# hongfz16/Garment4D

Hardware: AMD Instinct MI355X
Metric: point-cloud frames/s (FPS+ball_query+SA-MLP+LBS), B=8 N=8192 (higher is better)
Workload: dtype f32

## Files before the change

### garment4d_amd/_lib.py

```python
import ctypes
import os

_HERE = os.path.dirname(os.path.abspath(__file__))
LIB_PATH = os.environ.get("G4D_LIB_PATH") or os.path.join(_HERE, "lib", "libg4d_hip.so")

_vp = ctypes.c_void_p
_I = ctypes.c_int
_F = ctypes.c_float
_LL = ctypes.c_longlong

SIGNATURES = {
    "g4d_fps_f32": [_I, _I, _I, _vp, _vp, _vp, _vp],
    "g4d_fps_gather_f32": [_I, _I, _I, _vp, _vp, _vp, _vp, _vp],
    "g4d_gather_f32": [_I, _I, _I, _I, _vp, _vp, _vp, _vp],
    "g4d_gather_grad_f32": [_I, _I, _I, _I, _vp, _vp, _vp, _vp],
    "g4d_ball_query_f32": [_I, _I, _I, _F, _I, _vp, _vp, _vp, _vp],
    "g4d_ball_query_msg_f32": [_I, _I, _I, _I, _vp, _vp, _vp, _vp, _vp, _vp],
    "g4d_ball_query_boxes_f32": [_I, _I, _I, _I, _vp, _vp, _vp, _vp, _vp, _vp, _vp],
    "g4d_ball_query_lanes_f32": [_I, _I, _I, _I, _vp, _vp, _vp, _vp, _vp, _vp, _vp, _vp],
    "g4d_ball_query_lanes_qsort_bytes": [_I, _I],
    "g4d_ball_grid_bytes": [_I, _I],
    "g4d_ball_grid_build_f32": [_I, _I, _F, _vp, _vp, _vp],
    "g4d_ball_grid_query_f32": [_I, _I, _I, _I, _vp, _vp, _vp, _vp, _vp, _vp, _F, _vp],
    "g4d_ball_query_grid_f32": [_I, _I, _I, _I, _vp, _vp, _vp, _vp, _vp, _vp, _vp],
# ... 48 lines not shown
    "g4d_mlp_chain_table_f32": [ctypes.c_longlong, _I, _I, _I, _vp, _vp, _vp, _vp, _vp, _vp, _I, _I, _vp, _vp, _vp, _vp, _vp, _vp, _vp, _I, _I, _I, _vp, _I, _vp],
    "g4d_mlp_chain_group_table_f32": [ctypes.c_longlong, _I, _I, _I, _vp, _vp, _vp, _vp, _I, _I, _vp, _vp, _vp, _I, _vp, _vp, _vp, _vp, _vp, _vp, _I, _vp, _I, _I, _vp],
    "g4d_mlp_args_size": [],
    "g4d_mlp_run": [_I, _vp, _vp],
    "g4d_sa_table_supported": [ctypes.c_longlong, _I, _I, _I],
    "g4d_sa_table_ws_bytes": [ctypes.c_longlong, _I, _I, _I],
    "g4d_mlp_chain_group_table_ws_f32": [ctypes.c_longlong, _I, _I, _I, _vp, _vp, _vp, _vp, _I, _I, _vp, _vp, _vp, _I, _vp, _vp, _vp, _vp, _vp, _vp, _I, _vp, _I, _I, _vp,
                                         ctypes.c_longlong, _vp],
    "g4d_three_nn_cells_f32": [_I, _I, _I, _vp, _vp, _vp, _vp, _vp, _vp],
    "g4d_mlp_chain_interp_init_f32": [ctypes.c_longlong, _I, _I, _I, _vp, _vp, _I, _vp, _vp, _I, _vp, _vp, _vp, _vp, _vp, _vp, _vp, _I, _I, _I, _vp, _I, _vp],
    "g4d_three_nn_multi_f32": [_I, _I, _vp, _vp, _vp, _vp, _vp, _vp, _vp],
    "g4d_ball_query_msg2_f32": [_I, _I, _I, _I, _vp, _vp, _vp, _vp, _vp, _I, _I, _vp, _vp, _vp, _vp, _vp, _vp],
    "g4d_fps_gather_pair_supported": [_I, _I, _I],
    "g4d_fps_gather_pair_f32": [_I, _I, _I, _I, _vp, _vp, _vp, _vp, _vp, _vp],
    "g4d_sa_xyz_mlp3_pair_f32": [_I, _I, _I, _vp, _vp, _I, _vp, _I, _I, _vp, _vp, _I, _vp, _vp, _vp, _I, _vp, _vp, _vp, _I, _vp, _vp, _I, _I, _vp, _vp, _I, _vp, _vp, _vp, _I, _vp, _vp, _vp, _I, _vp, _vp, _I, _vp],
    "g4d_fps_gather_grid_f32": [_I, _I, _I, _vp, _vp, _vp, ctypes.c_float, _vp, _vp],
    "g4d_three_nn_cells_sorted_f32": [_I, _I, _I, _vp, _vp, _vp, _vp, _vp],
    "g4d_three_nn_pruned_supported": [_I, _I],
    "g4d_three_nn_pruned_ws_bytes": [_I],
    "g4d_three_nn_pruned_f32": [_I, _I, _I, _vp, _vp, _vp, _vp, _vp, _I, _vp, ctypes.c_longlong, _vp],
    "g4d_mlp_chain_table_cells_f32": [ctypes.c_longlong, _I, _I, _I, _vp, _vp, _vp, _vp, _vp, _vp, _vp, _I, _I, _vp, _vp, _vp, _vp, _vp, _vp, _vp, _I, _I, _I, _vp, _I, _vp],
    "g4d_search_multi_f32": [_I, _I, _I, _I, _vp, _vp, _vp, _vp, _vp, _I, _I, _vp, _vp, _vp, _vp, _vp, _I, _vp, _vp, _vp, _vp, _vp, _vp, _vp],
    "g4d_launch_group_begin": [],
    "g4d_launch_group_end": [_vp, _vp],
    "g4d_launch_group_abort": [],
    "g4d_lbs_one_supported": [_I, _I],
    "g4d_lbs_one_f32": [_I, _I, _I, _I, _I, _vp, _I, _vp, _vp, _vp, _vp, _vp, _vp, _vp, _vp, _vp, _vp, _vp],
    "g4d_lbs_mfma_supported": [_I, _I],
    "g4d_lbs_mfma_ws_bytes": [_I, _I],
    "g4d_lbs_mfma_f32": [_I, _I, _I, _I, _I, _vp, _I, _vp, _vp, _vp, _vp, _vp, _vp, _vp, _vp, _vp, _vp, _vp, ctypes.c_longlong, _vp],
# ... 2 lines not shown
    "g4d_segment_take_f32": [_I, _I, _I, _I, _vp, _vp, _vp, _vp],
    "g4d_vertex_normals_f32": [_I, _I, _vp, _vp, _vp, _vp, _vp, _vp],
    "g4d_spmm_axpy_rows_f32": [_I, _I, _I, _vp, _vp, _vp, _vp, _F, _vp, _vp],
    "g4d_jacobi_smooth_f32": [_I, _I, _I, _I, _F, _I, _vp, _vp, _vp, _vp, _vp, _vp],
    "g4d_gather_rows_f32": [_I, _I, _I, _I, _vp, _vp, _vp, _vp],
    "g4d_lbs_shape_f32": [_I, _I, _I, _vp, _I, _vp, _vp, _vp, _vp],
    "g4d_joint_regress_f32": [_I, _I, _I, _vp, _I, _vp, _vp, _vp],
    "g4d_rodrigues_f32": [_I, _vp, _vp, _vp],
    "g4d_rigid_transform_f32": [_I, _I, _I, _vp, _vp, _vp, _vp, _vp, _vp, _vp, _vp],
    "g4d_lbs_pose_skin_f32": [_I, _I, _I, _I, _vp, _vp, _vp, _vp, _I, _vp, _vp, _vp, _vp],
}

_lib = None


RESTYPES = {"g4d_mlp_args_size": ctypes.c_uint, "g4d_sa_table_ws_bytes": ctypes.c_longlong, "g4d_gcn_tile_meta_bytes": ctypes.c_longlong, "g4d_frag_bf16_elems": ctypes.c_longlong, "g4d_lbs_mfma_ws_bytes": ctypes.c_longlong, "g4d_three_nn_pruned_ws_bytes": ctypes.c_longlong, "g4d_temporal_attention_scratch_floats": ctypes.c_size_t, "g4d_ball_grid_bytes": ctypes.c_size_t, "g4d_ball_query_lanes_qsort_bytes": ctypes.c_size_t}


class G4DError(RuntimeError):
    pass


MLP_ARGS_VERSION = 1
MLP_STACK_F32, MLP_STACK_BF16, MLP_WAVE_F32, MLP_CHAIN_F32, MLP_CHAIN_BF16, MLP_CHAIN_BF16X3 = range(6)


class MlpArgs(ctypes.Structure):
    _fields_ = [("size", ctypes.c_uint), ("version", ctypes.c_uint), ("mode", _I), ("K0", _I), ("rows", ctypes.c_longlong),
                ("X", _vp), ("ldx", _I),
                ("N", _I), ("P", _I), ("S", _I), ("C", _I), ("use_xyz", _I), ("xyz", _vp), ("new_xyz", _vp), ("feats", _vp), ("idx", _vp),
                ("n", _I), ("m", _I), ("C2", _I), ("C1", _I), ("known_feats", _vp), ("skip", _vp), ("dist2", _vp), ("nn_idx", _vp),
# ... 105 lines not shown
```

### garment4d_amd/csrc/api.hip

```cpp
#include <stdarg.h>
#include <stddef.h>
#include <stdlib.h>
#include <string.h>

#include "g4d_common.h"

namespace g4d {
static thread_local char g_err[512] = "";

void set_error(const char *fmt, ...) {
    va_list ap;
    va_start(ap, fmt);
    vsnprintf(g_err, sizeof(g_err), fmt, ap);
    va_end(ap);
}

static int g_contract = -1;

static int parse_contract(const char *e) {
    if (!e || !*e) return G4D_CONTRACT_NVCC;
    if (!strcmp(e, "0") || !strcmp(e, "off") || !strcmp(e, "none")) return G4D_CONTRACT_OFF;
    if (!strcmp(e, "2") || !strcmp(e, "chain") || !strcmp(e, "inner")) return G4D_CONTRACT_CHAIN;
    return G4D_CONTRACT_NVCC;
}
// ... 4 lines not shown
    if (t_contract >= 0) return t_contract;
    int m = __atomic_load_n(&g_contract, __ATOMIC_RELAXED);
    if (m < 0) {
        m = parse_contract(getenv("G4D_DIST_CONTRACT"));
        __atomic_store_n(&g_contract, m, __ATOMIC_RELAXED);
    }
    return m;
}
}

namespace g4d {
namespace {
struct Tune { const char *key; long long value; int state; };
Tune g_tune[] = {{"sa_table_persistent", 0, 0}, {"sa_table_min_rows", 0, 0}, {"sa_table_128", 0, 0}, {"sa_table_oversub", 0, 0}, {"sa_table_dedup", 0, 0}, {"fp_table_persistent", 0, 0},
                 {"fp_table_min_rows", 0, 0}, {"gemm_tile", 0, 0}, {"gemm_tile_min_rows", 0, 0}, {"gemm_tile_min_cout", 0, 0}, {"gemm_tile_min_kpad", 0, 0}, {"fp_init_persistent", 0, 0}, {"fp_init_min_rows", 0, 0},
                 {"fp_head_bf16_persistent", 0, 0}, {"fp_head_bf16_min_rows", 0, 0}, {"sa_group_bf16_persistent", 0, 0}, {"sa_group_bf16_min_rows", 0, 0}};
}
struct ThreadTune { long long value; bool set; };
thread_local ThreadTune t_tune[sizeof(g_tune) / sizeof(g_tune[0])] = {};

long long tuning(const char *key, long long dflt) {
    int i = 0;
    for (Tune &t : g_tune) {
        const int slot = i++;
        if (strcmp(t.key, key)) continue;
        if (t_tune[slot].set) return t_tune[slot].value;
        int st = __atomic_load_n(&t.state, __ATOMIC_ACQUIRE);
        if (st == 0) {
            char env[64] = "G4D_";
            size_t n = 4;
            for (const char *c = key; *c && n + 1 < sizeof(env); ++c) env[n++] = (char)((*c >= 'a' && *c <= 'z') ? *c - 32 : *c);
// ... 32 lines not shown
    if (key) {
        int i = 0;
        for (g4d::Tune &t : g4d::g_tune) {
            const int slot = i++;
            if (!strcmp(t.key, key)) {
                g4d::t_tune[slot].value = value;
                g4d::t_tune[slot].set = set != 0;
                return G4D_OK;
            }
        }
    }
    g4d::set_error("g4d_tuning_set_thread: unknown key '%s'", key ? key : "(null)");
    return G4D_EINVAL;
}

extern "C" int g4d_version(void) { return 260;  }
extern "C" const char *g4d_last_error(void) { return g4d::g_err; }

extern "C" int g4d_get_distance_contraction(void) { return g4d::distance_contraction(); }
extern "C" int g4d_set_distance_contraction_thread(int mode) {
    const int prev = g4d::t_contract;
    if (mode < -1 || mode > G4D_CONTRACT_CHAIN) {
        g4d::set_error("g4d_set_distance_contraction_thread: mode %d is not -1 (no override) or one of G4D_CONTRACT_OFF/NVCC/CHAIN", mode);
        return -2;
    }
    g4d::t_contract = mode;
    return prev;
}

extern "C" int g4d_set_distance_contraction(int mode) {
    const int saved = g4d::t_contract;
// ... 97 lines not shown
```

### garment4d_amd/csrc/sa_xyz.hip

```cpp
#include <cstdlib>

#include "g4d_common.h"

namespace g4d {

typedef float f32x4 __attribute__((ext_vector_type(4)));

struct SaXyzArgs {
    int n, p, S, logS, pool;
    long long rows;
    const float *xyz, *new_xyz;
    const int *idx;
    const float *W1, *sc1, *sh1;
    int ldw1;
    const float *W2f, *sc2, *sh2;
    const float *W3f, *sc3, *sh3;
    int kst2, kst3;
    float *out;
    int ldo, col0;
};

struct __attribute__((packed, aligned(4))) F3s { float x, y, z; };
__device__ __forceinline__ F3s ld3(const float *base, unsigned elem) {
    return *reinterpret_cast<const F3s *>(reinterpret_cast<const char *>(base) + (elem << 2));
}

__device__ __forceinline__ float pool4_rows_max(float v0, float v1, float v2, float v3) {
    const auto a = __builtin_amdgcn_permlane16_swap(__float_as_uint(v0), __float_as_uint(v1), false, false);
    const auto b = __builtin_amdgcn_permlane16_swap(__float_as_uint(v2), __float_as_uint(v3), false, false);
    const float m01 = fmaxf(__uint_as_float(a[0]), __uint_as_float(a[1]));
    const float m23 = fmaxf(__uint_as_float(b[0]), __uint_as_float(b[1]));
    const auto c = __builtin_amdgcn_permlane32_swap(__float_as_uint(m01), __float_as_uint(m23), false, false);
    return fmaxf(__uint_as_float(c[0]), __uint_as_float(c[1]));
}

template <int C1, int C2, int C3, int LOGS, bool MAXP>
__device__ __forceinline__ void sa_xyz_body(const SaXyzArgs &a, int first, int stride) {
    constexpr int T1 = C1 / 16, T2 = C2 / 16, T3 = C3 / 16;
    constexpr int S = 1 << LOGS;
    static_assert(S == 16 || S == 32, "16 or 32 samples");
    static_assert(T3 == 2 || T3 == 4, "32 or 64 output channels");
    const int lane = threadIdx.x & 63;
    const int fi = lane & 15, fq = lane >> 4;
    float w1f[T1], s1[T1][4], h1s[T1][4];
#pragma unroll
    for (int ks = 0; ks < T1; ++ks) {
        const float w = a.W1[(ks * 16 + fi) * a.ldw1 + min(fq, 2)];
        w1f[ks] = fq < 3 ? w : 0.f;
#pragma unroll
        for (int e = 0; e < 4; ++e) {
            const int c = ks * 16 + fq * 4 + e;
// ... 9 lines not shown
#pragma unroll
    for (int ct = 0; ct < T3; ++ct)
#pragma unroll
        for (int ks = 0; ks < T2; ++ks) w3[ct][ks] = *reinterpret_cast<const f32x4 *>(a.W3f + ((size_t)(ct * a.kst3 + ks) * 64 + lane) * 4);
    f32x4 s2[T2], h2s[T2];
#pragma unroll
    for (int ct = 0; ct < T2; ++ct) {
        s2[ct] = *reinterpret_cast<const f32x4 *>(a.sc2 + ct * 16 + fq * 4);
        h2s[ct] = *reinterpret_cast<const f32x4 *>(a.sh2 + ct * 16 + fq * 4);
    }
    float s3[T3], h3s[T3];
#pragma unroll
    for (int ct = 0; ct < T3; ++ct) { s3[ct] = a.sc3[ct * 16 + fi]; h3s[ct] = a.sh3[ct * 16 + fi]; }

    const int rows = (int)a.rows;
    const int npass = (rows + 31) >> 5;
    struct Rows { float px[2], pq[2]; };
    int ivn[2];
    auto load_idx = [&](int pass, int (&v)[2]) {
#pragma unroll
        for (int mt = 0; mt < 2; ++mt) v[mt] = a.idx[min(min(pass, npass - 1) * 32 + mt * 16 + fi, rows - 1)];
    };
    const int nq = (int)(a.rows >> LOGS);
    auto load_rows = [&](int pass, const int (&v)[2], Rows &rw) {
        pass = min(pass, npass - 1);
#pragma unroll
        for (int mt = 0; mt < 2; ++mt) {
            const int qi = __builtin_amdgcn_readfirstlane(min((pass * 32 + mt * 16) >> LOGS, nq - 1));
            const int f = qi / a.p;
            rw.px[mt] = a.xyz[(unsigned)(f * a.n + v[mt]) * 3u + cfq];
            rw.pq[mt] = a.new_xyz[(unsigned)qi * 3u + cfq];
        }
    };
    auto do_pass = [&](int pass, const Rows &cur, Rows &fill, bool alive) {
        load_rows(pass + stride, ivn, fill);
        load_idx(pass + 2 * stride, ivn);
        __builtin_amdgcn_sched_barrier(0);
        const int row0 = pass * 32;
        f32x4 h1[2][T1];
#pragma unroll
        for (int mt = 0; mt < 2; ++mt) {
            const float d = cur.px[mt] - cur.pq[mt];
            const float comp = fq < 3 ? d : 0.f;
#pragma unroll
            for (int ks = 0; ks < T1; ++ks) {
                const f32x4 acc = __builtin_amdgcn_mfma_f32_16x16x4f32(w1f[ks], comp, (f32x4){0.f, 0.f, 0.f, 0.f}, 0, 0, 0);
#pragma unroll
                for (int e = 0; e < 4; ++e) h1[mt][ks][e] = fmaxf(__builtin_fmaf(acc[e], s1[ks][e], h1s[ks][e]), 0.f);
            }
// ... 20 lines not shown
                for (int r = 0; r < 4; ++r) h2[mt][ct][r] = fmaxf(__builtin_fmaf(h2[mt][ct][r], s2[ct][r], h2s[ct][r]), 0.f);
        f32x4 acc[2][T3];
#pragma unroll
        for (int mt = 0; mt < 2; ++mt)
#pragma unroll
            for (int ct = 0; ct < T3; ++ct) acc[mt][ct] = (f32x4){0.f, 0.f, 0.f, 0.f};
#pragma unroll
        for (int ks = 0; ks < T2; ++ks)
#pragma unroll
            for (int e = 0; e < 4; ++e)
#pragma unroll
                for (int mt = 0; mt < 2; ++mt)
#pragma unroll
                    for (int ct = 0; ct < T3; ++ct)
                        acc[mt][ct] = __builtin_amdgcn_mfma_f32_16x16x4f32(h2[mt][ks][e], w3[ct][ks][e], acc[mt][ct], 0, 0, 0);
        if constexpr (MAXP) {
            float v[2][T3];
#pragma unroll
            for (int mt = 0; mt < 2; ++mt)
#pragma unroll
                for (int ct = 0; ct < T3; ++ct) {
                    const float y0 = __builtin_fmaf(acc[mt][ct][0], s3[ct], h3s[ct]), y1 = __builtin_fmaf(acc[mt][ct][1], s3[ct], h3s[ct]),
                                y2 = __builtin_fmaf(acc[mt][ct][2], s3[ct], h3s[ct]), y3 = __builtin_fmaf(acc[mt][ct][3], s3[ct], h3s[ct]);
                    v[mt][ct] = fmaxf(fmaxf(y0, y1), fmaxf(y2, y3));
                }
            if constexpr (S == 32) {
                float x[T3];
#pragma unroll
                for (int ct = 0; ct < T3; ++ct) x[ct] = fmaxf(v[0][ct], v[1][ct]);
                float *o = a.out + (size_t)pass * a.ldo + a.col0;
                if constexpr (T3 == 4) {
// ... 66 lines not shown
        if (a.S == 16) sa_xyz_body<C1, C2, C3, 4, false>(a, first, stride);
        else sa_xyz_body<C1, C2, C3, 5, false>(a, first, stride);
    }
}

template <int C1, int C2, int C3>
__global__ void __launch_bounds__(256, 2) sa_xyz_kernel(const SaXyzArgs a) {
    sa_xyz_dispatch<C1, C2, C3>(a, blockIdx.x * 4 + __builtin_amdgcn_readfirstlane(threadIdx.x >> 6), gridDim.x * 4);
}

template <bool MAXP>
__global__ void __launch_bounds__(256, 2) sa_xyz_pair_kernel(const SaXyzArgs a0, const SaXyzArgs a1) {
    const int first = blockIdx.x * 4 + __builtin_amdgcn_readfirstlane(threadIdx.x >> 6), stride = gridDim.x * 4;
    sa_xyz_body<32, 32, 64, 5, MAXP>(a1, first, stride);
    sa_xyz_body<16, 16, 32, 4, MAXP>(a0, first, stride);
}

}

using namespace g4d;

extern "C" int g4d_sa_xyz_mlp3_supported(int c1, int c2, int c3, int nsample) {
    return ((c1 == 16 && c2 == 16 && c3 == 32) || (c1 == 32 && c2 == 32 && c3 == 64)) && (nsample == 16 || nsample == 32);
}

static int sa_xyz_fill(SaXyzArgs &a, int b, int n, int p, int nsample, const float *xyz, const float *new_xyz, const int *idx, int c1, int c2, int c3,
                       const float *W1, int ldw1, const float *scale1, const float *shift1, const float *W2_frag, int kpad2, const float *scale2,
                       const float *shift2, const float *W3_frag, int kpad3, const float *scale3, const float *shift3, int pool, float *out, int ldo,
                       int col0) {
    G4D_REQUIRE(b >= 0 && n > 0 && p >= 0, "g4d_sa_xyz_mlp3_f32: bad sizes");
    G4D_REQUIRE(g4d_sa_xyz_mlp3_supported(c1, c2, c3, nsample), "g4d_sa_xyz_mlp3_f32: widths %d-%d-%d over %d samples are not instantiated", c1, c2,
                c3, nsample);
    G4D_REQUIRE(pool == 1 || pool == 2, "g4d_sa_xyz_mlp3_f32: pool must be 1 (max) or 2 (avg)");
    const long long rows = (long long)b * p * nsample;
    G4D_REQUIRE(xyz && new_xyz && idx && W1 && scale1 && shift1 && W2_frag && scale2 && shift2 && W3_frag && scale3 && shift3 && out && ldw1 >= 3,
                "g4d_sa_xyz_mlp3_f32: null pointer");
    G4D_REQUIRE(ldo >= col0 + c3 && col0 >= 0, "g4d_sa_xyz_mlp3_f32: output window out of range");
    G4D_REQUIRE(rows < (1ll << 31) - 64 && (long long)b * n * 12 < (1ll << 32), "g4d_sa_xyz_mlp3_f32: needs rows < 2^31 and b*n*12 B < 4 GB");
    a.n = n; a.p = p; a.S = nsample; a.logS = nsample == 16 ? 4 : 5; a.pool = pool; a.rows = rows;
    a.xyz = xyz; a.new_xyz = new_xyz; a.idx = idx; a.W1 = W1; a.sc1 = scale1; a.sh1 = shift1; a.ldw1 = ldw1;
    G4D_REQUIRE(kpad2 % 16 == 0 && kpad2 >= c1 && kpad3 % 16 == 0 && kpad3 >= c2, "g4d_sa_xyz_mlp3_f32: Kpad of layers 2 / 3 must be multiples of 16 covering c1 / c2");
    a.W2f = W2_frag; a.sc2 = scale2; a.sh2 = shift2; a.W3f = W3_frag; a.sc3 = scale3; a.sh3 = shift3; a.kst2 = kpad2 / 16; a.kst3 = kpad3 / 16;
    a.out = out; a.ldo = ldo; a.col0 = col0;
    return G4D_OK;
}

extern "C" int g4d_sa_xyz_mlp3_pair_f32(int b, int n, int p, const float *xyz, const float *new_xyz, int pool, float *out, int ldo,
                                        int nsample0, const int *idx0, const float *W1_0, int ldw1_0, const float *scale1_0, const float *shift1_0,
                                        const float *W2_frag0, int kpad2_0, const float *scale2_0, const float *shift2_0, const float *W3_frag0,
                                        int kpad3_0, const float *scale3_0, const float *shift3_0, int col0_0,
                                        int nsample1, const int *idx1, const float *W1_1, int ldw1_1, const float *scale1_1, const float *shift1_1,
                                        const float *W2_frag1, int kpad2_1, const float *scale2_1, const float *shift2_1, const float *W3_frag1,
                                        int kpad3_1, const float *scale3_1, const float *shift3_1, int col0_1, g4d_stream_t stream) {
    SaXyzArgs a0, a1;
    if (int rc = sa_xyz_fill(a0, b, n, p, nsample0, xyz, new_xyz, idx0, 16, 16, 32, W1_0, ldw1_0, scale1_0, shift1_0, W2_frag0, kpad2_0, scale2_0, shift2_0,
                             W3_frag0, kpad3_0, scale3_0, shift3_0, pool, out, ldo, col0_0)) return rc;
    if (int rc = sa_xyz_fill(a1, b, n, p, nsample1, xyz, new_xyz, idx1, 32, 32, 64, W1_1, ldw1_1, scale1_1, shift1_1, W2_frag1, kpad2_1, scale2_1, shift2_1,
                             W3_frag1, kpad3_1, scale3_1, shift3_1, pool, out, ldo, col0_1)) return rc;
    if (a0.rows == 0) return G4D_OK;
    G4D_REQUIRE(nsample0 == 16 && nsample1 == 32, "g4d_sa_xyz_mlp3_pair_f32: scale 0 takes 16 samples, scale 1 takes 32");
    static const int bpc = [] { const char *e = getenv("G4D_SA_XYZ_BLOCKS_PER_CU"); return e && atoi(e) > 0 ? atoi(e) : 3; }();
    const long long want = ((a1.rows + 31) / 32 + 3) / 4;
    const unsigned grid = (unsigned)(want < 256 * bpc ? want : 256 * bpc);
    hipStream_t st = reinterpret_cast<hipStream_t>(stream);
    if (pool == 1) hipLaunchKernelGGL(sa_xyz_pair_kernel<true>, dim3(grid), dim3(256), 0, st, a0, a1);
    else hipLaunchKernelGGL(sa_xyz_pair_kernel<false>, dim3(grid), dim3(256), 0, st, a0, a1);
    return check_launch("g4d_sa_xyz_mlp3_pair_f32");
}

extern "C" int g4d_sa_xyz_mlp3_f32(int b, int n, int p, int nsample, const float *xyz, const float *new_xyz, const int *idx, int c1, int c2,
                                   int c3, const float *W1, int ldw1, const float *scale1, const float *shift1, const float *W2_frag, int kpad2,
                                   const float *scale2, const float *shift2, const float *W3_frag, int kpad3, const float *scale3, const float *shift3,
                                   int pool, float *out, int ldo, int col0, g4d_stream_t stream) {
    G4D_REQUIRE(b >= 0 && n > 0 && p >= 0, "g4d_sa_xyz_mlp3_f32: bad sizes");
    G4D_REQUIRE(g4d_sa_xyz_mlp3_supported(c1, c2, c3, nsample), "g4d_sa_xyz_mlp3_f32: widths %d-%d-%d over %d samples are not instantiated", c1, c2,
                c3, nsample);
    G4D_REQUIRE(pool == 1 || pool == 2, "g4d_sa_xyz_mlp3_f32: pool must be 1 (max) or 2 (avg)");
    const long long rows = (long long)b * p * nsample;
    if (rows == 0) return G4D_OK;
    G4D_REQUIRE(xyz && new_xyz && idx && W1 && scale1 && shift1 && W2_frag && scale2 && shift2 && W3_frag && scale3 && shift3 && out && ldw1 >= 3,
                "g4d_sa_xyz_mlp3_f32: null pointer");
    G4D_REQUIRE(ldo >= col0 + c3 && col0 >= 0, "g4d_sa_xyz_mlp3_f32: output window out of range");
    G4D_REQUIRE(rows < (1ll << 31) - 64 && (long long)b * n * 12 < (1ll << 32), "g4d_sa_xyz_mlp3_f32: needs rows < 2^31 and b*n*12 B < 4 GB");
    SaXyzArgs a;
    a.n = n; a.p = p; a.S = nsample; a.logS = nsample == 16 ? 4 : 5; a.pool = pool; a.rows = rows;
    a.xyz = xyz; a.new_xyz = new_xyz; a.idx = idx; a.W1 = W1; a.sc1 = scale1; a.sh1 = shift1; a.ldw1 = ldw1;
    G4D_REQUIRE(kpad2 % 16 == 0 && kpad2 >= c1 && kpad3 % 16 == 0 && kpad3 >= c2, "g4d_sa_xyz_mlp3_f32: Kpad of layers 2 / 3 must be multiples of 16 covering c1 / c2");
    a.W2f = W2_frag; a.sc2 = scale2; a.sh2 = shift2; a.W3f = W3_frag; a.sc3 = scale3; a.sh3 = shift3; a.kst2 = kpad2 / 16; a.kst3 = kpad3 / 16;
    a.out = out; a.ldo = ldo; a.col0 = col0;
    const long long npass = (rows + 31) / 32, want = (npass + 3) / 4;
    static const int bpc = [] { const char *e = getenv("G4D_SA_XYZ_BLOCKS_PER_CU"); return e && atoi(e) > 0 ? atoi(e) : 3; }();
    const unsigned grid = (unsigned)(want < 256 * bpc ? want : 256 * bpc);
    hipStream_t st = reinterpret_cast<hipStream_t>(stream);
    if (c1 == 16) hipLaunchKernelGGL((sa_xyz_kernel<16, 16, 32>), dim3(grid), dim3(256), 0, st, a);
    else hipLaunchKernelGGL((sa_xyz_kernel<32, 32, 64>), dim3(grid), dim3(256), 0, st, a);
    return check_launch("g4d_sa_xyz_mlp3_f32");
}
```

### garment4d_amd/fused.py

```python
import contextlib
import ctypes
import os

import torch
import torch.nn as nn

from . import _lib
from . import pointnet2_utils as PU
from .tuning import current as _T

_KC = 32
_BN = 64


def _ptr(t):
    return 0 if t is None else t.data_ptr()


def _chk(t, dtype=torch.float32):
    assert t.is_cuda and t.dtype == dtype and t.is_contiguous(), "fused path needs contiguous HIP tensors"
    return t


class PackedLayer:
# ... 603 lines not shown
        out = torch.empty((B, P, ctot), dtype=torch.float32, device=xyz.device)
        col0 = 0
        if idxs is None:
            idxs = ball_query_msg([g.radius for g in sa.groupers], [g.nsample for g in sa.groupers], xyz, new_xyz, grid=grid)
        if (_T().use_sa_xyz and _T().sa_xyz_pair and C == 0 and len(packed) == 2 and current_precision() == "fp32" and B * N * 12 < 2 ** 32
                and all(int(g.use_xyz) for g in sa.groupers) and all(len(L_) == 3 and all(L.relu for L in L_) for L_ in packed)
                and [L.Cout for L in packed[0]] == [16, 16, 32] and [L.Cout for L in packed[1]] == [32, 32, 64]
                and [g.nsample for g in sa.groupers] == [16, 32]):
            args = []
            c0 = 0
            for g, L_, idx in zip(sa.groupers, packed, idxs):
                L1, L2, L3 = L_
                args += [g.nsample, idx.data_ptr(), L1.W.data_ptr(), L1.Kpad, L1.scale.data_ptr(), L1.shift.data_ptr(), L2.Wf.data_ptr(), L2.Kpad,
                         L2.scale.data_ptr(), L2.shift.data_ptr(), L3.Wf.data_ptr(), L3.Kpad, L3.scale.data_ptr(), L3.shift.data_ptr(), c0]
                c0 += L3.Cout
            _lib.call("g4d_sa_xyz_mlp3_pair_f32", B, N, P, xyz.data_ptr(), new_xyz.data_ptr(), pool, out.data_ptr(), out.shape[-1], *args, stream)
            return new_xyz, out
        tab_scales = [k for k, (g, layers) in enumerate(zip(sa.groupers, packed))
                      if sa_table_fits(layers, C, int(g.use_xyz), pool, g.nsample, B * N, B * P * g.nsample)]
        table, toffs = sa_level_table(sa, packed, feats_pm, tab_scales) if tab_scales else (None, [])
        grouped = 1 < len(packed) <= 4 and len(tab_scales) == len(packed)
        with (launch_group() if grouped else contextlib.nullcontext()):
            for k, (grouper, layers, idx) in enumerate(zip(sa.groupers, packed, idxs)):
                S = grouper.nsample
                use_xyz = int(grouper.use_xyz)
                assert use_xyz or feats_pm is not None
                tb = None
                if k in tab_scales:
                    c0, wxT = toffs[tab_scales.index(k)]
                    tb = (table, c0, wxT)
                sa_scale_mlp(xyz, new_xyz, feats_pm, idx, layers, use_xyz, pool, out, col0, table=tb)
# ... 263 lines not shown
```

### garment4d_amd/tuning.py

```python
import contextlib
import contextvars
import dataclasses
import os
from typing import Mapping, Tuple


def _env_flag(name, default):
    return os.environ.get(name, "1" if default else "0") != "0"


def _env_int(name, default):
    return int(os.environ.get(name, str(default)))


NATIVE_KEYS = ("sa_table_persistent", "sa_table_min_rows", "sa_table_128", "sa_table_oversub", "sa_table_dedup", "fp_table_persistent", "fp_table_min_rows", "gemm_tile",
               "gemm_tile_min_rows", "gemm_tile_min_cout", "gemm_tile_min_kpad", "fp_init_persistent", "fp_init_min_rows",
               "fp_head_bf16_persistent", "fp_head_bf16_min_rows", "sa_group_bf16_persistent", "sa_group_bf16_min_rows")


@dataclasses.dataclass(frozen=True)
class Tuning:
    use_wave: bool = True
    use_stack: bool = True
    use_chain: bool = True
    stream_gemm: bool = True
    bf16_min_rows: int = 0
    overlap_sampling: bool = False
    lanes_sort: bool = False
    coherent_lanes: bool = False
    grid_min_n: int = 4096
    fps_pair: bool = True
    bq_multi: bool = True
# ... 89 lines not shown
```

### include/g4d.h

```cpp
#ifndef G4D_H
#define G4D_H

#include <stddef.h>

#ifdef __cplusplus
extern "C" {
#endif

typedef struct ihipStream_t *g4d_stream_t;

#define G4D_OK 0
#define G4D_EINVAL 10001

int g4d_version(void);
const char *g4d_last_error(void);

#define G4D_CONTRACT_OFF 0
#define G4D_CONTRACT_NVCC 1
#define G4D_CONTRACT_CHAIN 2
int g4d_get_distance_contraction(void);
int g4d_set_distance_contraction(int mode);
int g4d_set_distance_contraction_thread(int mode);


// ... 247 lines not shown
                            const float *xyz0, int *const *idx0, int n1, int m1, const float *radii1, const int *nsamples1,
                            const float *new_xyz1, const float *xyz1, int *const *idx1, g4d_stream_t stream);

int g4d_fps_gather_pair_supported(int n, int m1, int m2);
int g4d_fps_gather_pair_f32(int b, int n, int m1, int m2, const float *xyz, int *idx1, float *new_xyz1, int *idx2, float *new_xyz2,
                            g4d_stream_t stream);

int g4d_sa_xyz_mlp3_pair_f32(int b, int n, int p, const float *xyz, const float *new_xyz, int pool, float *out, int ldo,
                             int nsample0, const int *idx0, const float *W1_0, int ldw1_0, const float *scale1_0, const float *shift1_0,
                             const float *W2_frag0, int kpad2_0, const float *scale2_0, const float *shift2_0, const float *W3_frag0, int kpad3_0,
                             const float *scale3_0, const float *shift3_0, int col0_0,
                             int nsample1, const int *idx1, const float *W1_1, int ldw1_1, const float *scale1_1, const float *shift1_1,
                             const float *W2_frag1, int kpad2_1, const float *scale2_1, const float *shift2_1, const float *W3_frag1, int kpad3_1,
                             const float *scale3_1, const float *shift3_1, int col0_1, g4d_stream_t stream);

int g4d_three_nn_cells_sorted_f32(int b, int n, int m, const void *unknown_grid, const float *known, float *dist2, int *idx, g4d_stream_t stream);

int g4d_three_nn_pruned_supported(int n, int m);
long long g4d_three_nn_pruned_ws_bytes(int b);
int g4d_three_nn_pruned_f32(int b, int n, int m, const float *unknown, const void *unknown_grid, const float *known, float *dist2, int *idx,
                            int sorted_out, void *ws, long long ws_bytes, g4d_stream_t stream);
int g4d_mlp_chain_table_cells_f32(long long rows, int n, int m, int C2, const float *table, const float *dist2, const int *nn_idx,
                                  const void *unknown_grid, const float *pre_scale, const float *pre_shift, float *in_tap, int in_tap_ld,
                                  int nlayers, const float *const *W, const float *const *scale, const float *const *shift, const int *Kpad,
                                  const int *Cout, const int *relu, float *out, int ldo, int col0, int tap_layer, float *tap_out, int tap_ld,
                                  g4d_stream_t stream);

int g4d_search_multi_f32(int b, int nscales, int n0, int m0, const float *radii0, const int *nsamples0, const float *new_xyz0, const float *xyz0,
                         int *const *idx0, int n1, int m1, const float *radii1, const int *nsamples1, const float *new_xyz1, const float *xyz1,
                         int *const *idx1, int nn_count, const int *nn_n, const int *nn_m, const float *const *nn_unknown,
// ... 58 lines not shown
```

Baseline: 52980.

## Pack deduplicated ball-query neighbours before the fused SA xyz MLP with pooled max

Adds a pre-pass kernel that removes the repeated padded neighbour indices ball query leaves in each group. It compacts the surviving rows into per-chunk packed arrays, each with a group key marking its centre and group end. The fused three-layer SA MLP kernel then processes only these live rows and max-pools across packed rows through a per-wave LDS buffer, writing each centre's output when its group ends. This is meant to skip MLP work on duplicate samples when ball query finds fewer neighbours than nsample. The cost is an extra kernel launch, a per-call workspace allocation, and more complex pooling logic.

Measured after the change: 53040 (median of 6 runs). No clear change (+0.1%).

```diff
diff --git a/garment4d_amd/_lib.py b/garment4d_amd/_lib.py
--- a/garment4d_amd/_lib.py
+++ b/garment4d_amd/_lib.py
@@ -86,6 +86,8 @@
     "g4d_fps_gather_pair_supported": [_I, _I, _I],
     "g4d_fps_gather_pair_f32": [_I, _I, _I, _I, _vp, _vp, _vp, _vp, _vp, _vp],
     "g4d_sa_xyz_mlp3_pair_f32": [_I, _I, _I, _vp, _vp, _I, _vp, _I, _I, _vp, _vp, _I, _vp, _vp, _vp, _I, _vp, _vp, _vp, _I, _vp, _vp, _I, _I, _vp, _vp, _I, _vp, _vp, _vp, _I, _vp, _vp, _vp, _I, _vp, _vp, _I, _vp],
+    "g4d_sa_xyz_mlp3_pair_ws_f32": [_I, _I, _I, _vp, _vp, _I, _vp, _I, _I, _vp, _vp, _I, _vp, _vp, _vp, _I, _vp, _vp, _vp, _I, _vp, _vp, _I, _I, _vp, _vp, _I, _vp, _vp, _vp, _I, _vp, _vp, _vp, _I, _vp, _vp, _I, _vp, ctypes.c_longlong, _vp],
+    "g4d_sa_xyz_pair_ws_bytes": [_I, _I, _I],
     "g4d_fps_gather_grid_f32": [_I, _I, _I, _vp, _vp, _vp, ctypes.c_float, _vp, _vp],
     "g4d_three_nn_cells_sorted_f32": [_I, _I, _I, _vp, _vp, _vp, _vp, _vp],
     "g4d_three_nn_pruned_supported": [_I, _I],
@@ -118,7 +120,7 @@
 _lib = None
 
 
-RESTYPES = {"g4d_mlp_args_size": ctypes.c_uint, "g4d_sa_table_ws_bytes": ctypes.c_longlong, "g4d_gcn_tile_meta_bytes": ctypes.c_longlong, "g4d_frag_bf16_elems": ctypes.c_longlong, "g4d_lbs_mfma_ws_bytes": ctypes.c_longlong, "g4d_three_nn_pruned_ws_bytes": ctypes.c_longlong, "g4d_temporal_attention_scratch_floats": ctypes.c_size_t, "g4d_ball_grid_bytes": ctypes.c_size_t, "g4d_ball_query_lanes_qsort_bytes": ctypes.c_size_t}
+RESTYPES = {"g4d_mlp_args_size": ctypes.c_uint, "g4d_sa_xyz_pair_ws_bytes": ctypes.c_longlong, "g4d_sa_table_ws_bytes": ctypes.c_longlong, "g4d_gcn_tile_meta_bytes": ctypes.c_longlong, "g4d_frag_bf16_elems": ctypes.c_longlong, "g4d_lbs_mfma_ws_bytes": ctypes.c_longlong, "g4d_three_nn_pruned_ws_bytes": ctypes.c_longlong, "g4d_temporal_attention_scratch_floats": ctypes.c_size_t, "g4d_ball_grid_bytes": ctypes.c_size_t, "g4d_ball_query_lanes_qsort_bytes": ctypes.c_size_t}
 
 
 class G4DError(RuntimeError):
diff --git a/garment4d_amd/csrc/api.hip b/garment4d_amd/csrc/api.hip
--- a/garment4d_amd/csrc/api.hip
+++ b/garment4d_amd/csrc/api.hip
@@ -42,7 +42,7 @@
 struct Tune { const char *key; long long value; int state; };
 Tune g_tune[] = {{"sa_table_persistent", 0, 0}, {"sa_table_min_rows", 0, 0}, {"sa_table_128", 0, 0}, {"sa_table_oversub", 0, 0}, {"sa_table_dedup", 0, 0}, {"fp_table_persistent", 0, 0},
                  {"fp_table_min_rows", 0, 0}, {"gemm_tile", 0, 0}, {"gemm_tile_min_rows", 0, 0}, {"gemm_tile_min_cout", 0, 0}, {"gemm_tile_min_kpad", 0, 0}, {"fp_init_persistent", 0, 0}, {"fp_init_min_rows", 0, 0},
-                 {"fp_head_bf16_persistent", 0, 0}, {"fp_head_bf16_min_rows", 0, 0}, {"sa_group_bf16_persistent", 0, 0}, {"sa_group_bf16_min_rows", 0, 0}};
+                 {"fp_head_bf16_persistent", 0, 0}, {"fp_head_bf16_min_rows", 0, 0}, {"sa_group_bf16_persistent", 0, 0}, {"sa_group_bf16_min_rows", 0, 0}, {"sa_pack", 0, 0}};
 }
 struct ThreadTune { long long value; bool set; };
 thread_local ThreadTune t_tune[sizeof(g_tune) / sizeof(g_tune[0])] = {};
@@ -105,7 +105,7 @@
     return G4D_EINVAL;
 }
 
-extern "C" int g4d_version(void) { return 260;  }
+extern "C" int g4d_version(void) { return 270;  }
 extern "C" const char *g4d_last_error(void) { return g4d::g_err; }
 
 extern "C" int g4d_get_distance_contraction(void) { return g4d::distance_contraction(); }
diff --git a/garment4d_amd/csrc/sa_xyz.hip b/garment4d_amd/csrc/sa_xyz.hip
--- a/garment4d_amd/csrc/sa_xyz.hip
+++ b/garment4d_amd/csrc/sa_xyz.hip
@@ -18,6 +18,8 @@
     int kst2, kst3;
     float *out;
     int ldo, col0;
+    const int *prow, *gkey, *npass;
+    int nchunk;
 };
 
 struct __attribute__((packed, aligned(4))) F3s { float x, y, z; };
@@ -34,7 +36,76 @@
     return fmaxf(__uint_as_float(c[0]), __uint_as_float(c[1]));
 }
 
-template <int C1, int C2, int C3, int LOGS, bool MAXP>
+constexpr int kKeyLast = (int)0x80000000u, kKeyCentre = 0x7fffffff, kKeyPad = 0x7fffffff, kPoolLd = 80;
+constexpr int kChunkSlack = 64;
+constexpr int kSaPackDefault = 1;
+
+__host__ __device__ __forceinline__ long long pack_q0(int c, int nchunk, long long nq) { return (long long)c * nq / nchunk; }
+__host__ __device__ __forceinline__ int pack_rbase(int c, int nchunk, int nq, int S) { return (int)(pack_q0(c, nchunk, nq) * S) + c * kChunkSlack; }
+__host__ __device__ __forceinline__ long long pack_rows(long long nq, int S, int nchunk) { return nq * S + (long long)nchunk * kChunkSlack; }
+
+template <int LOGS>
+__device__ __forceinline__ void sa_pack_chunk(int c, int nq, int n, int p, int nchunk, const int *__restrict__ idx, int *__restrict__ prow,
+                                              int *__restrict__ gkey, int *__restrict__ npass) {
+    constexpr int S = 1 << LOGS, UPL = 64 / S, K = 16;
+    const int lane = threadIdx.x & 63;
+    const float inv_p = 1.f / (float)p;
+    const int q0 = (int)pack_q0(c, nchunk, nq), q1 = (int)pack_q0(c + 1, nchunk, nq);
+    const int r0 = pack_rbase(c, nchunk, nq, S);
+    const int seg = lane >> LOGS, j = lane & (S - 1);
+    const unsigned long long below = (1ull << lane) - 1ull;
+    int R = 0;
+    for (int qb = q0; qb < q1; qb += UPL * K) {
+        int vv[K];
+#pragma unroll
+        for (int k = 0; k < K; ++k) {
+            const int q = qb + k * UPL + seg;
+            vv[k] = q < q1 ? idx[(long long)q * S + j] : 0;
+        }
+#pragma unroll
+        for (int k = 0; k < K; ++k) {
+            const int q = qb + k * UPL + seg;
+            const bool valid = q < q1;
+            const int v = vv[k];
+            const int h = __builtin_amdgcn_ds_bpermute((lane & ~(S - 1)) << 2, v);
+            const bool live = valid && (j == 0 || v != h);
+            const unsigned long long m = __builtin_amdgcn_ballot_w64(live);
+            int cnt = 0, off = 0, acc = 0;
+#pragma unroll
+            for (int s = 0; s < UPL; ++s) {
+                const int cs = __builtin_popcountll((m >> (s * S)) & (S == 64 ? ~0ull : ((1ull << S) - 1ull)));
+                if (seg == s) { cnt = cs; off = acc; }
+                acc += (cs + 3) & ~3;
+            }
+            const int lr = (cnt + 3) & ~3;
+            const int base = r0 + R + off;
+            int f = (int)((float)q * inv_p);
+            f -= f * p > q;
+            f += (f + 1) * p <= q;
+            if (!valid) f = 0;
+            if (live) prow[base + __builtin_popcountll(m & below & (((1ull << S) - 1ull) << (seg * S)))] = f * n + v;
+            if (valid && j < lr - cnt) prow[base + cnt + j] = f * n + h;
+            if (valid && j < lr / 4) gkey[(base >> 2) + j] = q | (j == lr / 4 - 1 ? kKeyLast : 0);
+            R += acc;
+        }
+    }
+    const int np = (R + 31) >> 5;
+    if (lane < np * 32 - R) prow[r0 + R + lane] = 0;
+    if (lane < np * 8 - R / 4) gkey[(r0 + R) / 4 + lane] = kKeyPad;
+    if (lane == 0) npass[c] = np;
+}
+
+__global__ void __launch_bounds__(256) sa_pack_kernel(const SaXyzArgs a0, const SaXyzArgs a1, int s0) {
+    const int c = blockIdx.x * 4 + (threadIdx.x >> 6);
+    const int nq = (int)(a0.rows >> a0.logS);
+    if (s0 + (int)blockIdx.y == 0) {
+        if (c < a0.nchunk) sa_pack_chunk<4>(c, nq, a0.n, a0.p, a0.nchunk, a0.idx, const_cast<int *>(a0.prow), const_cast<int *>(a0.gkey), const_cast<int *>(a0.npass));
+    } else {
+        if (c < a1.nchunk) sa_pack_chunk<5>(c, nq, a1.n, a1.p, a1.nchunk, a1.idx, const_cast<int *>(a1.prow), const_cast<int *>(a1.gkey), const_cast<int *>(a1.npass));
+    }
+}
+
+template <int C1, int C2, int C3, int LOGS, bool MAXP, bool PACK = false>
 __device__ __forceinline__ void sa_xyz_body(const SaXyzArgs &a, int first, int stride) {
     constexpr int T1 = C1 / 16, T2 = C2 / 16, T3 = C3 / 16;
     constexpr int S = 1 << LOGS;
@@ -74,15 +145,39 @@
     for (int ct = 0; ct < T3; ++ct) { s3[ct] = a.sc3[ct * 16 + fi]; h3s[ct] = a.sh3[ct * 16 + fi]; }
 
     const int rows = (int)a.rows;
-    const int npass = (rows + 31) >> 5;
+    int npass = (rows + 31) >> 5;
+    int rbase = 0;
+    if constexpr (PACK) {
+        npass = __builtin_amdgcn_readfirstlane(a.npass[first]);
+        rbase = pack_rbase(first, a.nchunk, rows >> LOGS, S);
+        first = 0; stride = 1;
+        if (npass == 0) return;
+    }
     struct Rows { float px[2], pq[2]; };
-    int ivn[2];
-    auto load_idx = [&](int pass, int (&v)[2]) {
-#pragma unroll
-        for (int mt = 0; mt < 2; ++mt) v[mt] = a.idx[min(min(pass, npass - 1) * 32 + mt * 16 + fi, rows - 1)];
+    int ivn[PACK ? 4 : 2];
+    const int nq = (int)(a.rows >> LOGS);
+    auto load_idx = [&](int pass, auto &v) {
+        if constexpr (PACK) {
+            const int r = rbase + min(pass, npass - 1) * 32 + fi;
+#pragma unroll
+            for (int mt = 0; mt < 2; ++mt) {
+                v[mt] = a.prow[r + mt * 16];
+                v[2 + mt] = min(a.gkey[(r + mt * 16) >> 2] & kKeyCentre, nq - 1);
+            }
+        } else {
+#pragma unroll
+            for (int mt = 0; mt < 2; ++mt) v[mt] = a.idx[min(min(pass, npass - 1) * 32 + mt * 16 + fi, rows - 1)];
+        }
     };
-    const int nq = (int)(a.rows >> LOGS);
-    auto load_rows = [&](int pass, const int (&v)[2], Rows &rw) {
+    auto load_rows = [&](int pass, const auto &v, Rows &rw) {
+        if constexpr (PACK) {
+#pragma unroll
+            for (int mt = 0; mt < 2; ++mt) {
+                rw.px[mt] = a.xyz[(unsigned)v[mt] * 3u + cfq];
+                rw.pq[mt] = a.new_xyz[(unsigned)v[2 + mt] * 3u + cfq];
+            }
+            return;
+        }
         pass = min(pass, npass - 1);
 #pragma unroll
         for (int mt = 0; mt < 2; ++mt) {
@@ -92,7 +187,11 @@
             rw.pq[mt] = a.new_xyz[(unsigned)qi * 3u + cfq];
         }
     };
+    float pm = 0.f;
+    int pq_run = -1;
     auto do_pass = [&](int pass, const Rows &cur, Rows &fill, bool alive) {
+        int kv = 0;
+        if constexpr (PACK) kv = a.gkey[(rbase >> 2) + min(pass, npass - 1) * 8 + (lane & 7)];
         load_rows(pass + stride, ivn, fill);
         load_idx(pass + 2 * stride, ivn);
         __builtin_amdgcn_sched_barrier(0);
@@ -143,7 +242,30 @@
 #pragma unroll
                     for (int ct = 0; ct < T3; ++ct)
                         acc[mt][ct] = __builtin_amdgcn_mfma_f32_16x16x4f32(h2[mt][ks][e], w3[ct][ks][e], acc[mt][ct], 0, 0, 0);
-        if constexpr (MAXP) {
+        if constexpr (PACK) {
+            __shared__ float s_pool[4][8 * kPoolLd];
+            float *sp = s_pool[threadIdx.x >> 6];
+            if (alive) {
+#pragma unroll
+                for (int mt = 0; mt < 2; ++mt)
+#pragma unroll
+                    for (int ct = 0; ct < T3; ++ct) {
+                        const float y0 = __builtin_fmaf(acc[mt][ct][0], s3[ct], h3s[ct]), y1 = __builtin_fmaf(acc[mt][ct][1], s3[ct], h3s[ct]),
+                                    y2 = __builtin_fmaf(acc[mt][ct][2], s3[ct], h3s[ct]), y3 = __builtin_fmaf(acc[mt][ct][3], s3[ct], h3s[ct]);
+                        sp[(mt * 4 + fq) * kPoolLd + ct * 16 + fi] = fmaxf(fmaxf(y0, y1), fmaxf(y2, y3));
+                    }
+                __builtin_amdgcn_fence(__ATOMIC_RELEASE, "wavefront");
+                __builtin_amdgcn_fence(__ATOMIC_ACQUIRE, "wavefront");
+#pragma unroll
+                for (int g = 0; g < 8; ++g) {
+                    const float x = sp[g * kPoolLd + lane];
+                    const int key = __builtin_amdgcn_readlane(kv, g), q = key & kKeyCentre;
+                    pm = q == pq_run ? fmaxf(pm, x) : x;
+                    pq_run = q;
+                    if ((key & kKeyLast) && lane < C3) a.out[(size_t)q * a.ldo + a.col0 + lane] = fmaxf(pm, 0.f);
+                }
+            }
+        } else if constexpr (MAXP) {
             float v[2][T3];
 #pragma unroll
             for (int mt = 0; mt < 2; ++mt)
@@ -240,6 +362,13 @@
     const int first = blockIdx.x * 4 + __builtin_amdgcn_readfirstlane(threadIdx.x >> 6), stride = gridDim.x * 4;
     sa_xyz_body<32, 32, 64, 5, MAXP>(a1, first, stride);
     sa_xyz_body<16, 16, 32, 4, MAXP>(a0, first, stride);
+}
+
+template <bool P0, bool P1>
+__global__ void __launch_bounds__(256, 3) sa_xyz_pair_packed_kernel(const SaXyzArgs a0, const SaXyzArgs a1) {
+    const int first = blockIdx.x * 4 + __builtin_amdgcn_readfirstlane(threadIdx.x >> 6), stride = gridDim.x * 4;
+    sa_xyz_body<32, 32, 64, 5, true, P1>(a1, first, stride);
+    sa_xyz_body<16, 16, 32, 4, true, P0>(a0, first, stride);
 }
 
 }
@@ -268,7 +397,72 @@
     G4D_REQUIRE(kpad2 % 16 == 0 && kpad2 >= c1 && kpad3 % 16 == 0 && kpad3 >= c2, "g4d_sa_xyz_mlp3_f32: Kpad of layers 2 / 3 must be multiples of 16 covering c1 / c2");
     a.W2f = W2_frag; a.sc2 = scale2; a.sh2 = shift2; a.W3f = W3_frag; a.sc3 = scale3; a.sh3 = shift3; a.kst2 = kpad2 / 16; a.kst3 = kpad3 / 16;
     a.out = out; a.ldo = ldo; a.col0 = col0;
+    a.prow = a.gkey = a.npass = nullptr; a.nchunk = 0;
     return G4D_OK;
+}
+
+static unsigned sa_xyz_pair_grid(long long rows1) {
+    static const int bpc = [] { const char *e = getenv("G4D_SA_XYZ_BLOCKS_PER_CU"); return e && atoi(e) > 0 ? atoi(e) : 3; }();
+    const long long want = ((rows1 + 31) / 32 + 3) / 4;
+    return (unsigned)(want < 256 * bpc ? want : 256 * bpc);
+}
+
+static long long align256(long long x) { return (x + 255) & ~255ll; }
+static long long sa_pack_scale_bytes(long long nq, int S, int nchunk) {
+    const long long r = pack_rows(nq, S, nchunk);
+    return align256(4 * r) + align256(r) + align256(4ll * nchunk);
+}
+static int sa_pack_mask() { return (int)(tuning("sa_pack", kSaPackDefault) & 3); }
+static long long sa_pack_bytes(int b, int p, int pool) {
+    const long long nq = (long long)b * p;
+    const int mask = sa_pack_mask();
+    if (pool != 1 || nq <= 0 || !mask || nq * 32 >= (1ll << 31) - 64) return 0;
+    const int nchunk = (int)sa_xyz_pair_grid(nq * 32) * 4;
+    return ((mask & 1) ? sa_pack_scale_bytes(nq, 16, nchunk) : 0) + ((mask & 2) ? sa_pack_scale_bytes(nq, 32, nchunk) : 0);
+}
+
+extern "C" long long g4d_sa_xyz_pair_ws_bytes(int b, int p, int pool) { return sa_pack_bytes(b, p, pool); }
+
+extern "C" int g4d_sa_xyz_mlp3_pair_ws_f32(int b, int n, int p, const float *xyz, const float *new_xyz, int pool, float *out, int ldo,
+                                        int nsample0, const int *idx0, const float *W1_0, int ldw1_0, const float *scale1_0, const float *shift1_0,
+                                        const float *W2_frag0, int kpad2_0, const float *scale2_0, const float *shift2_0, const float *W3_frag0,
+                                        int kpad3_0, const float *scale3_0, const float *shift3_0, int col0_0,
+                                        int nsample1, const int *idx1, const float *W1_1, int ldw1_1, const float *scale1_1, const float *shift1_1,
+                                        const float *W2_frag1, int kpad2_1, const float *scale2_1, const float *shift2_1, const float *W3_frag1,
+                                        int kpad3_1, const float *scale3_1, const float *shift3_1, int col0_1, void *ws, long long ws_bytes,
+                                        g4d_stream_t stream) {
+    SaXyzArgs a0, a1;
+    if (int rc = sa_xyz_fill(a0, b, n, p, nsample0, xyz, new_xyz, idx0, 16, 16, 32, W1_0, ldw1_0, scale1_0, shift1_0, W2_frag0, kpad2_0, scale2_0, shift2_0,
+                             W3_frag0, kpad3_0, scale3_0, shift3_0, pool, out, ldo, col0_0)) return rc;
+    if (int rc = sa_xyz_fill(a1, b, n, p, nsample1, xyz, new_xyz, idx1, 32, 32, 64, W1_1, ldw1_1, scale1_1, shift1_1, W2_frag1, kpad2_1, scale2_1, shift2_1,
+                             W3_frag1, kpad3_1, scale3_1, shift3_1, pool, out, ldo, col0_1)) return rc;
+    if (a0.rows == 0) return G4D_OK;
+    G4D_REQUIRE(nsample0 == 16 && nsample1 == 32, "g4d_sa_xyz_mlp3_pair_f32: scale 0 takes 16 samples, scale 1 takes 32");
+    const unsigned grid = sa_xyz_pair_grid(a1.rows);
+    hipStream_t st = reinterpret_cast<hipStream_t>(stream);
+    const long long need = sa_pack_bytes(b, p, pool);
+    if (ws && need > 0 && ws_bytes >= need) {
+        const int mask = sa_pack_mask(), nchunk = (int)grid * 4, nq = b * p;
+        char *w = static_cast<char *>(ws);
+        SaXyzArgs *sc[2] = {&a0, &a1};
+        for (int s = 0; s < 2; ++s) {
+            if (!(mask >> s & 1)) continue;
+            SaXyzArgs &a = *sc[s];
+            const long long r = pack_rows(nq, a.S, nchunk);
+            a.prow = reinterpret_cast<int *>(w); w += align256(4 * r);
+            a.gkey = reinterpret_cast<int *>(w); w += align256(r);
+            a.npass = reinterpret_cast<int *>(w); w += align256(4ll * nchunk);
+            a.nchunk = nchunk;
+        }
+        hipLaunchKernelGGL(sa_pack_kernel, dim3(grid, mask == 3 ? 2 : 1), dim3(256), 0, st, a0, a1, mask == 2 ? 1 : 0);
+        if (mask == 1) hipLaunchKernelGGL((sa_xyz_pair_packed_kernel<true, false>), dim3(grid), dim3(256), 0, st, a0, a1);
+        else if (mask == 2) hipLaunchKernelGGL((sa_xyz_pair_packed_kernel<false, true>), dim3(grid), dim3(256), 0, st, a0, a1);
+        else hipLaunchKernelGGL((sa_xyz_pair_packed_kernel<true, true>), dim3(grid), dim3(256), 0, st, a0, a1);
+        return check_launch("g4d_sa_xyz_mlp3_pair_ws_f32");
+    }
+    if (pool == 1) hipLaunchKernelGGL(sa_xyz_pair_kernel<true>, dim3(grid), dim3(256), 0, st, a0, a1);
+    else hipLaunchKernelGGL(sa_xyz_pair_kernel<false>, dim3(grid), dim3(256), 0, st, a0, a1);
+    return check_launch("g4d_sa_xyz_mlp3_pair_f32");
 }
 
 extern "C" int g4d_sa_xyz_mlp3_pair_f32(int b, int n, int p, const float *xyz, const float *new_xyz, int pool, float *out, int ldo,
@@ -278,20 +472,10 @@
                                         int nsample1, const int *idx1, const float *W1_1, int ldw1_1, const float *scale1_1, const float *shift1_1,
                                         const float *W2_frag1, int kpad2_1, const float *scale2_1, const float *shift2_1, const float *W3_frag1,
                                         int kpad3_1, const float *scale3_1, const float *shift3_1, int col0_1, g4d_stream_t stream) {
-    SaXyzArgs a0, a1;
-    if (int rc = sa_xyz_fill(a0, b, n, p, nsample0, xyz, new_xyz, idx0, 16, 16, 32, W1_0, ldw1_0, scale1_0, shift1_0, W2_frag0, kpad2_0, scale2_0, shift2_0,
-                             W3_frag0, kpad3_0, scale3_0, shift3_0, pool, out, ldo, col0_0)) return rc;
-    if (int rc = sa_xyz_fill(a1, b, n, p, nsample1, xyz, new_xyz, idx1, 32, 32, 64, W1_1, ldw1_1, scale1_1, shift1_1, W2_frag1, kpad2_1, scale2_1, shift2_1,
-                             W3_frag1, kpad3_1, scale3_1, shift3_1, pool, out, ldo, col0_1)) return rc;
-    if (a0.rows == 0) return G4D_OK;
-    G4D_REQUIRE(nsample0 == 16 && nsample1 == 32, "g4d_sa_xyz_mlp3_pair_f32: scale 0 takes 16 samples, scale 1 takes 32");
-    static const int bpc = [] { const char *e = getenv("G4D_SA_XYZ_BLOCKS_PER_CU"); return e && atoi(e) > 0 ? atoi(e) : 3; }();
-    const long long want = ((a1.rows + 31) / 32 + 3) / 4;
-    const unsigned grid = (unsigned)(want < 256 * bpc ? want : 256 * bpc);
-    hipStream_t st = reinterpret_cast<hipStream_t>(stream);
-    if (pool == 1) hipLaunchKernelGGL(sa_xyz_pair_kernel<true>, dim3(grid), dim3(256), 0, st, a0, a1);
-    else hipLaunchKernelGGL(sa_xyz_pair_kernel<false>, dim3(grid), dim3(256), 0, st, a0, a1);
-    return check_launch("g4d_sa_xyz_mlp3_pair_f32");
+    return g4d_sa_xyz_mlp3_pair_ws_f32(b, n, p, xyz, new_xyz, pool, out, ldo, nsample0, idx0, W1_0, ldw1_0, scale1_0, shift1_0, W2_frag0, kpad2_0,
+                                       scale2_0, shift2_0, W3_frag0, kpad3_0, scale3_0, shift3_0, col0_0, nsample1, idx1, W1_1, ldw1_1, scale1_1,
+                                       shift1_1, W2_frag1, kpad2_1, scale2_1, shift2_1, W3_frag1, kpad3_1, scale3_1, shift3_1, col0_1, nullptr, 0,
+                                       stream);
 }
 
 extern "C" int g4d_sa_xyz_mlp3_f32(int b, int n, int p, int nsample, const float *xyz, const float *new_xyz, const int *idx, int c1, int c2,
@@ -314,6 +498,7 @@
     G4D_REQUIRE(kpad2 % 16 == 0 && kpad2 >= c1 && kpad3 % 16 == 0 && kpad3 >= c2, "g4d_sa_xyz_mlp3_f32: Kpad of layers 2 / 3 must be multiples of 16 covering c1 / c2");
     a.W2f = W2_frag; a.sc2 = scale2; a.sh2 = shift2; a.W3f = W3_frag; a.sc3 = scale3; a.sh3 = shift3; a.kst2 = kpad2 / 16; a.kst3 = kpad3 / 16;
     a.out = out; a.ldo = ldo; a.col0 = col0;
+    a.prow = a.gkey = a.npass = nullptr; a.nchunk = 0;
     const long long npass = (rows + 31) / 32, want = (npass + 3) / 4;
     static const int bpc = [] { const char *e = getenv("G4D_SA_XYZ_BLOCKS_PER_CU"); return e && atoi(e) > 0 ? atoi(e) : 3; }();
     const unsigned grid = (unsigned)(want < 256 * bpc ? want : 256 * bpc);
diff --git a/garment4d_amd/fused.py b/garment4d_amd/fused.py
--- a/garment4d_amd/fused.py
+++ b/garment4d_amd/fused.py
@@ -641,7 +641,10 @@
                 args += [g.nsample, idx.data_ptr(), L1.W.data_ptr(), L1.Kpad, L1.scale.data_ptr(), L1.shift.data_ptr(), L2.Wf.data_ptr(), L2.Kpad,
                          L2.scale.data_ptr(), L2.shift.data_ptr(), L3.Wf.data_ptr(), L3.Kpad, L3.scale.data_ptr(), L3.shift.data_ptr(), c0]
                 c0 += L3.Cout
-            _lib.call("g4d_sa_xyz_mlp3_pair_f32", B, N, P, xyz.data_ptr(), new_xyz.data_ptr(), pool, out.data_ptr(), out.shape[-1], *args, stream)
+            nws = int(_lib.lib().g4d_sa_xyz_pair_ws_bytes(B, P, pool))
+            ws = torch.empty((nws + 3) // 4, dtype=torch.int32, device=xyz.device) if nws > 0 else None
+            _lib.call("g4d_sa_xyz_mlp3_pair_ws_f32", B, N, P, xyz.data_ptr(), new_xyz.data_ptr(), pool, out.data_ptr(), out.shape[-1], *args,
+                      _ptr(ws), nws, stream)
             return new_xyz, out
         tab_scales = [k for k, (g, layers) in enumerate(zip(sa.groupers, packed))
                       if sa_table_fits(layers, C, int(g.use_xyz), pool, g.nsample, B * N, B * P * g.nsample)]
diff --git a/garment4d_amd/tuning.py b/garment4d_amd/tuning.py
--- a/garment4d_amd/tuning.py
+++ b/garment4d_amd/tuning.py
@@ -15,7 +15,7 @@
 
 NATIVE_KEYS = ("sa_table_persistent", "sa_table_min_rows", "sa_table_128", "sa_table_oversub", "sa_table_dedup", "fp_table_persistent", "fp_table_min_rows", "gemm_tile",
                "gemm_tile_min_rows", "gemm_tile_min_cout", "gemm_tile_min_kpad", "fp_init_persistent", "fp_init_min_rows",
-               "fp_head_bf16_persistent", "fp_head_bf16_min_rows", "sa_group_bf16_persistent", "sa_group_bf16_min_rows")
+               "fp_head_bf16_persistent", "fp_head_bf16_min_rows", "sa_group_bf16_persistent", "sa_group_bf16_min_rows", "sa_pack")
 
 
 @dataclasses.dataclass(frozen=True)
diff --git a/include/g4d.h b/include/g4d.h
--- a/include/g4d.h
+++ b/include/g4d.h
@@ -285,6 +285,15 @@
                              const float *W2_frag1, int kpad2_1, const float *scale2_1, const float *shift2_1, const float *W3_frag1, int kpad3_1,
                              const float *scale3_1, const float *shift3_1, int col0_1, g4d_stream_t stream);
 
+long long g4d_sa_xyz_pair_ws_bytes(int b, int p, int pool);
+int g4d_sa_xyz_mlp3_pair_ws_f32(int b, int n, int p, const float *xyz, const float *new_xyz, int pool, float *out, int ldo,
+                                int nsample0, const int *idx0, const float *W1_0, int ldw1_0, const float *scale1_0, const float *shift1_0,
+                                const float *W2_frag0, int kpad2_0, const float *scale2_0, const float *shift2_0, const float *W3_frag0, int kpad3_0,
+                                const float *scale3_0, const float *shift3_0, int col0_0,
+                                int nsample1, const int *idx1, const float *W1_1, int ldw1_1, const float *scale1_1, const float *shift1_1,
+                                const float *W2_frag1, int kpad2_1, const float *scale2_1, const float *shift2_1, const float *W3_frag1, int kpad3_1,
+                                const float *scale3_1, const float *shift3_1, int col0_1, void *ws, long long ws_bytes, g4d_stream_t stream);
+
 int g4d_three_nn_cells_sorted_f32(int b, int n, int m, const void *unknown_grid, const float *known, float *dist2, int *idx, g4d_stream_t stream);
 
 int g4d_three_nn_pruned_supported(int n, int m);
```
